# jw3il/graph-marl

Hardware: AMD Instinct MI355X
Metric: env-steps/sec (routing, --netmon, 20-node graphs) at 1/2/4/8 MI355X (higher is better)
Workload: dtype f32 (GEMMs: 3xf16-split MFMA, A low piece scaled 2^12, f32 accumulate); 1 GPU; routing rollout --netmon (NetMon K=1, H=128, enc 512,256, lstm, sum) + DQN 512,256 eps-greedy, random 20-node topologies, episode 50 steps; n_env_per_gpu=4096, n_nodes=20, n_data=20, gemm_form=x3, parallelism=dp1 (env shards, no rollout collective), stream_groups=2, graph_steps=10, resets_in_window=43

## Files before the change

### graph-marl_amd/_lib.py

```python
import ctypes as C
import os

import torch

HERE = os.path.dirname(os.path.abspath(__file__))
LIB_PATH = os.environ.get("GM_LIB") or os.path.join(HERE, "lib", "libgraphmarl_amd.so")

GM_OK = 0
GM_ERR_UNSUPPORTED = -5
GM_INFO_FIELDS = 9
INFO_KEYS = ["looped", "throughput", "dropped", "blocked", "n_delays", "sum_delays", "n_arrived",
             "sum_delays_arrived", "sum_spr"]
TOPO_FIXED, TOPO_RANDOM, TOPO_LIST, TOPO_SEQUENTIAL = 0, 1, 2, 3
GM_EVAL_FIELDS = 5
EVAL_KEYS = ["total_edge_load", "occupied_edges", "packets_on_edges", "total_packet_size", "sum_packet_distances"]

EXPORTS = [
    "gm_last_error", "gm_version", "gm_env_create", "gm_env_destroy", "gm_env_dims", "gm_env_reset",
    "gm_env_step", "gm_env_observe", "gm_env_topology", "gm_env_final_info", "gm_policy_egreedy", "gm_env_policy_step",
    "gm_env_get_state", "gm_env_set_state", "gm_build_seed_list", "gm_mp_aggregate", "gm_mp_aggregate_rows", "gm_mp_aggregate_bwd", "gm_leaky_bwd", "gm_netmon_readout",
    "gm_netmon_readout_bwd", "gm_netmon_readout_bwd_sym", "gm_lstm_pointwise", "gm_lstm_pointwise_bwd", "gm_linear_f32", "gm_gemm_f32",
    "gm_simple_create", "gm_simple_destroy", "gm_simple_reset", "gm_simple_step",
    "gm_simple_observe", "gm_simple_policy_egreedy", "gm_simple_get_state", "gm_env_set_topology",
    "gm_policy_shortest_path", "gm_env_first_hops", "gm_routing_node_encoder", "gm_gemm_x3", "gm_gemm_x3_head", "gm_absmax_scale", "gm_absmax_scale_rows", "gm_gemm_x3_wgrad", "gm_gemm_x3_wgrad2", "gm_absmax_finish",
    "gm_gemm_pack_x3", "gm_gemm_pack_x3_bytes", "gm_gemm_range_status",
    "gm_pcg64_seed", "gm_pcg64_choice", "gm_lnlstm_pointwise", "gm_agent_attention", "gm_agent_comm",
    "gm_gemm_x3_dgrad", "gm_lstm_cell_bwd", "gm_qhead_bwd", "gm_netmon_readout_ld", "gm_routing_node_encoder_bits", "gm_gather_records",
    "gm_lnlstm_fwd", "gm_lnlstm_bwd", "gm_gru_pointwise", "gm_gru_bwd", "gm_act_bwd", "gm_build_info",
    "gm_act_fwd", "gm_act_bwd_z", "gm_obs_from_gemm", "gm_encoder_x3", "gm_step_mse_blocks", "gm_step_mse",
    "gm_step_mse_bwd", "gm_gru_cell_fwd", "gm_gru_cell_bwd", "gm_lnlstm_cell_bwd", "gm_agent_comm_bwd",
    "gm_agent_attention_bwd", "gm_agent_attention_kl", "gm_netmon_global_rows", "gm_netmon_global_bwd",
]
TUNING_EXPORTS = ["gm_gemm_set_tile", "gm_gemm_set_wgrad", "gm_gemm_set_mfma", "gm_gemm_set_dgrad", "gm_gemm_form",
                  "gm_last_kernel", "gm_last_lnlstm_pw", "gm_gemm_kernel_name"]

GEMM_MODE = os.environ.get("GM_GEMM", "x3")
if GEMM_MODE not in ("x3", "f32"):
    raise ValueError(f"GM_GEMM must be 'x3' or 'f32', not {GEMM_MODE!r}")

class EnvConfig(C.Structure):
    _fields_ = [
        ("n_env", C.c_int32), ("n_nodes", C.c_int32), ("n_data", C.c_int32), ("env_var", C.c_int32),
        ("congestion", C.c_int32), ("action_mask", C.c_int32), ("ttl", C.c_int32), ("topo_mode", C.c_int32),
        ("topo_seed", C.c_int64), ("seed_list", C.POINTER(C.c_int64)), ("n_seed_list", C.c_int32),
        ("excluded", C.POINTER(C.c_int64)), ("n_excluded", C.c_int32), ("device", C.c_int32),
        ("k", C.c_int32),
    ]


class ObsBuffers(C.Structure):
    _fields_ = [("obs", C.c_void_p), ("obs_row_stride", C.c_int64), ("node_obs", C.c_void_p),
                ("agent_node", C.c_void_p), ("agent_adj", C.c_void_p), ("obs_gemm", C.c_void_p),
                ("obs_gemm_stride", C.c_int64)]


class StepDetail(C.Structure):
    _fields_ = [("done_steps", C.c_void_p), ("done_opt", C.c_void_p), ("success", C.c_void_p), ("eval", C.c_void_p)]


class EnvState(C.Structure):
    _fields_ = [(k, C.c_void_p) for k in [
        "now", "target", "edge", "time", "ttl", "start", "spw", "agent_steps", "size", "visited", "amask",
        "loads", "topo_seed", "topo_reps", "edge_a", "edge_b", "edge_len", "nbr_edge", "apsp", "rng_key",
        "rng_pos", "seq_index"]]


class PCG64(C.Structure):
# ... 61 lines not shown
def lib():
    global _lib
    if _lib is not None:
        return _lib
    if not os.path.exists(LIB_PATH):
        raise GMError(f"{LIB_PATH} not built: run `make -C graph-marl_amd/csrc` (or __graft_entry__.build())")
    L = C.CDLL(LIB_PATH)
    vp, i32, i64 = C.c_void_p, C.c_int32, C.c_int64
    L.gm_last_error.restype = C.c_char_p
    L.gm_env_create.argtypes = [C.POINTER(EnvConfig), vp, C.POINTER(vp)]
    L.gm_env_destroy.argtypes = [vp]
    L.gm_env_dims.argtypes = [vp] + [C.POINTER(i32)] * 5
    L.gm_env_reset.argtypes = [vp, vp, C.POINTER(ObsBuffers), vp]
    L.gm_env_step.argtypes = [vp, vp, vp, vp, vp, C.POINTER(StepDetail), C.POINTER(ObsBuffers), vp]
    L.gm_env_observe.argtypes = [vp, C.POINTER(ObsBuffers), vp]
    L.gm_env_topology.argtypes = [vp, vp, vp, vp, vp, vp]
    L.gm_env_final_info.argtypes = [vp, vp, vp]
    L.gm_policy_egreedy.argtypes = [vp, vp, C.c_double, vp, vp]
    L.gm_env_policy_step.argtypes = [vp, vp, C.c_double, vp, vp, vp, vp, C.POINTER(StepDetail), C.POINTER(ObsBuffers),
                                     vp]
    L.gm_env_get_state.argtypes = [vp, C.POINTER(EnvState)]
    L.gm_env_set_state.argtypes = [vp, C.POINTER(EnvState)]
    L.gm_build_seed_list.argtypes = [i32, i64, i32, vp, i32, i32, vp]
    L.gm_mp_aggregate.argtypes = [vp, vp, i32, i32, i32, i32, i32, vp, vp]
    L.gm_mp_aggregate_rows.argtypes = [vp, C.c_int64, vp, i32, i32, i32, i32, i32, vp, C.c_int64, vp]
    L.gm_leaky_bwd.argtypes = [vp, vp, C.c_int64, i32, C.c_float, vp, vp, i32, vp, vp]
    L.gm_mp_aggregate_bwd.argtypes = [vp, vp, i32, i32, i32, i32, i32, vp, vp]
    L.gm_netmon_readout.argtypes = [vp, vp, vp, vp, i32, i32, i32, i32, i32, vp, i64, vp]
    L.gm_netmon_readout_bwd.argtypes = [vp, i64, vp, vp, i32, i32, i32, i32, i32, vp, vp, vp]
    L.gm_lstm_pointwise.argtypes = [vp, vp, i32, i32, vp, vp, vp, vp]
    L.gm_lstm_pointwise_bwd.argtypes = [vp, vp, vp, vp, vp, i32, i32, vp, vp, vp, vp]
    L.gm_linear_f32.argtypes = [vp, i64, vp, i64, vp, i32, i32, i32, i32, vp, i64, vp]
    L.gm_gemm_set_tile.argtypes = [i32]
    L.gm_gemm_set_wgrad.argtypes = [i32]
    L.gm_gemm_set_mfma.argtypes = [i32]
    L.gm_gemm_set_dgrad.argtypes = [i32]
    L.gm_lstm_cell_bwd.argtypes = [C.POINTER(LSTMBwdArgs), vp]
    L.gm_qhead_bwd.argtypes = [vp, i64, i32, vp, i64, vp, i64, i64, i32, i32, vp, i64, vp, vp, vp, i32, vp, vp]
    L.gm_netmon_readout_ld.argtypes = [vp, i64, vp, i64, vp, vp, i32, i32, i32, i32, i32, vp, i64, vp]
    L.gm_routing_node_encoder_bits.argtypes = [vp, i64, vp, i32, i32, vp, vp, i32, i32, vp, i64, vp, i64, vp]
    L.gm_env_set_topology.argtypes = [vp, i32, i64, vp, i32, i32]
    L.gm_policy_shortest_path.argtypes = [vp, vp, vp]
    L.gm_env_first_hops.argtypes = [vp, vp, vp]
    L.gm_agent_attention.argtypes = [vp, vp, vp, i64, vp, i32, i32, i32, i32, i32, vp, i64, vp, vp]
    L.gm_agent_comm.argtypes = [vp, i64, vp, i32, i32, i32, vp, i64, vp]
    L.gm_gemm_pack_x3_bytes.argtypes = [i32, i32]
    L.gm_gemm_pack_x3_bytes.restype = i64
    L.gm_gemm_pack_x3.argtypes = [vp, i64, i32, i32, vp, vp, vp]
    L.gm_routing_node_encoder.argtypes = [vp, i64, vp, i32, i32, vp, vp, i32, i32, vp, i64, vp]
    L.gm_gemm_range_status.argtypes = [C.POINTER(i32), i32]
    L.gm_pcg64_seed.argtypes = [C.c_uint64, C.POINTER(PCG64)]
    L.gm_pcg64_choice.argtypes = [vp, i64, i64, vp, vp]
    L.gm_gather_records.argtypes = [vp, i64, i64, vp, vp, i32, i64, i64, vp, vp]
    L.gm_lnlstm_pointwise.argtypes = [vp, i64, vp, i64] + [vp] * 7 + [i32, i32, C.c_float, vp, i64, vp, i64, vp]
    newer = {
        "gm_lnlstm_fwd": [vp, i64, vp, i64, vp, i64] + [vp] * 7 + [i32, i32, C.c_float, vp, i64, vp, i64, vp, vp],
        "gm_lnlstm_bwd": [vp, i64, vp, i64, vp, i64] + [vp] * 8 + [vp, i64, vp, i64, i32, i32, i32, vp, i64, vp, i64, vp,
                                                                   i64, vp, vp],
        "gm_gru_pointwise": [vp, i64, vp, i64, vp, i64, i32, i32, vp, i64, vp],
        "gm_gru_bwd": [vp, i64, vp, i64, vp, i64, vp, i64, i32, i32, vp, i64, vp, i64, vp, i64, vp],
        "gm_act_bwd": [vp, vp, C.c_int64, i32, i32, vp, vp, i32, vp, vp],
        "gm_act_fwd": [vp, C.c_int64, i32, i32, vp, vp],
        "gm_act_bwd_z": [vp, vp, C.c_int64, i32, i32, vp, vp, i32, vp, vp],
        "gm_obs_from_gemm": [vp, i64, i64, i32, vp, i64, vp],
        "gm_step_mse_blocks": [i64],
        "gm_step_mse": [vp, vp, i64, i32, vp, vp],
# ... 167 lines not shown
```

### graph-marl_amd/csrc/gm_device.hpp

```cpp
#pragma once
#include <hip/hip_runtime.h>
#include <stdint.h>

void gm_set_last_kernel(const char* name);

namespace gm {

constexpr int WAVE = 64;
constexpr int MT_N = 624;
constexpr int MT_M = 397;
constexpr int MAX_NODES = 128;
constexpr int MAX_AGENTS = 64;
constexpr int MAX_KNBR = 8;
constexpr int MAX_EDGES = MAX_NODES * 3 / 2;
constexpr int RNG_BUF = 256;

__device__ __forceinline__ int lane_id() { return threadIdx.x; }

__device__ __forceinline__ int readlane(int v, int l) { return __builtin_amdgcn_readlane(v, l); }
__device__ __forceinline__ uint32_t readlane_u(uint32_t v, int l) {
    return (uint32_t)__builtin_amdgcn_readlane((int)v, l);
}
__device__ __forceinline__ double readlane_f64(double v, int l) {
    uint64_t b = __double_as_longlong(v);
    uint32_t lo = readlane_u((uint32_t)b, l), hi = readlane_u((uint32_t)(b >> 32), l);
    return __longlong_as_double((long long)(((uint64_t)hi << 32) | lo));
}
__device__ __forceinline__ uint64_t readlane_u64(uint64_t v, int l) {
    uint32_t lo = readlane_u((uint32_t)v, l), hi = readlane_u((uint32_t)(v >> 32), l);
    return ((uint64_t)hi << 32) | lo;
}
__device__ __forceinline__ uint64_t ballot(bool p) { return __ballot(p); }

__device__ __forceinline__ bool bit128(const uint64_t* m, int v) { return (m[v >> 6] >> (v & 63)) & 1ull; }
__device__ __forceinline__ void set128(uint64_t* m, int v) { m[v >> 6] |= 1ull << (v & 63); }

__device__ __forceinline__ uint64_t wave_or_u64(uint64_t v) {
    uint32_t lo = (uint32_t)v, hi = (uint32_t)(v >> 32);
#pragma unroll
    for (int m = 1; m < WAVE; m <<= 1) {
        lo |= (uint32_t)__shfl_xor((int)lo, m);
        hi |= (uint32_t)__shfl_xor((int)hi, m);
    }
    return ((uint64_t)hi << 32) | lo;
}
__device__ __forceinline__ int wave_sum_i32(int v) {
#pragma unroll
    for (int m = 1; m < WAVE; m <<= 1) v += __shfl_xor(v, m);
    return v;
}

__device__ __forceinline__ uint32_t mt_temper(uint32_t y) {
    y ^= (y >> 11);
    y ^= (y << 7) & 0x9d2c5680u;
    y ^= (y << 15) & 0xefc60000u;
    y ^= (y >> 18);
    return y;
}

__device__ __forceinline__ uint32_t mt_mix(uint32_t a, uint32_t b, uint32_t m) {
    uint32_t y = (a & 0x80000000u) | (b & 0x7fffffffu);
    return m ^ (y >> 1) ^ ((0u - (y & 1u)) & 0x9908b0dfu);
}

__device__ __forceinline__ void mt_twist_lds(uint32_t* k) {
    const int l = lane_id();
    for (int s = 0; s < MT_N; s += WAVE) {
        int i = s + l;
        uint32_t a = 0, b = 0, m = 0;
        if (i < MT_N) {
            a = k[i];
            b = k[i == MT_N - 1 ? 0 : i + 1];
            m = k[i < MT_N - MT_M ? i + MT_M : i - (MT_N - MT_M)];
        }
        __syncthreads();
        if (i < MT_N) k[i] = mt_mix(a, b, m);
        __syncthreads();
    }
}

__device__ __forceinline__ void mt_seed_lds(uint32_t* k, uint32_t seed, int n = MT_N) {
    if (lane_id() == 0) {
        uint32_t v = seed;
        k[0] = v;
        for (int i = 1; i < n; i++) {
            v = 1812433253u * (v ^ (v >> 30)) + (uint32_t)i;
            k[i] = v;
        }
    }
    __syncthreads();
}

__device__ __forceinline__ uint32_t mask_for(uint32_t rng) {
    uint32_t m = rng;
    m |= m >> 1; m |= m >> 2; m |= m >> 4; m |= m >> 8; m |= m >> 16;
    return m;
}

struct MainRng {
    uint32_t* g;
    uint32_t* buf;
    uint32_t* tmp;
    int cur, pos, has_next;
    int n, k;

    __device__ void twist_next() {
        const int l = lane_id();
        const uint32_t* src = g + cur * MT_N;
        for (int i = l; i < MT_N; i += WAVE) tmp[i] = src[i];
        __syncthreads();
        mt_twist_lds(tmp);
        uint32_t* dst = g + (1 - cur) * MT_N;
        for (int i = l; i < MT_N; i += WAVE) dst[i] = tmp[i];
        __syncthreads();
        has_next = 1;
    }
    __device__ void commit() {
        pos += k;
        n = 0;
        k = 0;
        if (pos >= MT_N && has_next) {
            pos -= MT_N;
            cur = 1 - cur;
            has_next = 0;
        }
    }
    __device__ void prefetch(int want) {
        commit();
        if (want > RNG_BUF) want = RNG_BUF;
        if (pos + want > MT_N && !has_next) twist_next();
        int avail = (MT_N - pos) + (has_next ? MT_N : 0);
        if (want > avail) want = avail;
        const int l = lane_id();
        for (int i = l; i < want; i += WAVE) {
            int o = pos + i;
            uint32_t w = o < MT_N ? g[cur * MT_N + o] : g[(1 - cur) * MT_N + (o - MT_N)];
            buf[i] = mt_temper(w);
        }
        __syncthreads();
        n = want;
    }
    __device__ __forceinline__ uint32_t next32() {
        if (k >= n) prefetch(RNG_BUF);
        return buf[k++];
    }
    __device__ __forceinline__ int64_t randint(int64_t high) {
        uint32_t rng = (uint32_t)(high - 1);
        if (rng == 0) return 0;
        uint32_t m = mask_for(rng), v;
        for (int guard = 0; (v = (next32() & m)) > rng; guard++)
            if (guard > 4096) return 0;
        return (int64_t)v;
    }
    __device__ __forceinline__ double random() {
        int32_t a = (int32_t)(next32() >> 5), b = (int32_t)(next32() >> 6);
        return (a * 67108864.0 + b) / 9007199254740992.0;
    }
};

struct LocalRng {
    uint32_t* key;
    int pos;
    int lim = MT_N;
    uint32_t sd = 0;
    __device__ void seed(uint32_t s) {
        mt_seed_lds(key, s);
        pos = MT_N;
        lim = MT_N;
        sd = s;
    }
    __device__ void seed_partial(uint32_t s, int w) {
        mt_seed_lds(key, s, MT_M + w);
        const int l = lane_id();
        for (int c = 0; c < w; c += WAVE) {
            const int i = c + l;
            uint32_t a = 0, b = 0, m = 0;
            if (i < w) {
                a = key[i];
                b = key[i + 1];
                m = key[i + MT_M];
            }
            __syncthreads();
            if (i < w) key[i] = mt_mix(a, b, m);
            __syncthreads();
        }
        pos = 0;
        lim = w;
        sd = s;
    }
    __device__ __forceinline__ uint32_t next32() {
        if (pos == MT_N) {
            mt_twist_lds(key);
            pos = 0;
        }
        if (pos >= lim) {
            mt_seed_lds(key, sd);
            mt_twist_lds(key);
            lim = MT_N;
        }
        return mt_temper(key[pos++]);
    }
    __device__ __forceinline__ int64_t randint(int64_t high) {
        uint32_t rng = (uint32_t)(high - 1);
        if (rng == 0) return 0;
        uint32_t m = mask_for(rng), v;
        for (int guard = 0; (v = (next32() & m)) > rng; guard++)
            if (guard > 4096) return 0;
        return (int64_t)v;
    }
};

}
```

### graph-marl_amd/csrc/gm_env.hip

```cpp
#include <hip/hip_runtime.h>

#include <algorithm>
#include <cstdio>
#include <cstring>
#include <string>
#include <vector>

#include "../../include/graph_marl_amd.h"
#include "gm_device.hpp"

using namespace gm;

namespace {
thread_local std::string g_err;
}

extern "C" const char* gm_last_error(void) { return g_err.c_str(); }
extern "C" int gm_version(void) { return 1; }

int gm_fail(int code, const std::string& msg) {
    g_err = msg;
    return code;
}

// ... 20 lines not shown
    uint64_t* visited;
    uint8_t* amask;
    double* load;
    uint32_t* mt;
    int32_t *mt_cur, *mt_pos, *mt_has_next;
    int32_t* err;
};

struct gm_env {
    gm_env_config cfg;
    std::vector<int64_t> list, excl;
    EnvDev d;
    std::vector<void*> allocs;
    int device;
};

namespace {

template <int NC>
struct EnvLds {
    int32_t now[MAX_AGENTS], target[MAX_AGENTS], edge[MAX_AGENTS], time[MAX_AGENTS];
    double size[MAX_AGENTS];
    double load[NC * 3 / 2];
    uint8_t nbr[NC * 3], nbr_edge[NC * 3];
    uint8_t ea[NC * 3 / 2], eb[NC * 3 / 2], elen[NC * 3 / 2];
    uint64_t nbrmask[NC][2];
    int8_t kn[MAX_AGENTS][MAX_KNBR];
    float node_cnt[NC], node_load[NC];
    alignas(16) uint32_t rbuf[RNG_BUF];
    uint32_t rtmp[MT_N];
};
constexpr int STG_FLOATS = RNG_BUF + MT_N;

template <class ES>
__device__ void load_topology_lds(const EnvDev& d, int env, ES& s) {
    const int l = lane_id();
    const int N = d.N, E = d.E;
    for (int i = l; i < N * 3; i += WAVE) {
        s.nbr[i] = (uint8_t)d.nbr[(size_t)env * N * 3 + i];
        s.nbr_edge[i] = (uint8_t)d.nbr_edge[(size_t)env * N * 3 + i];
    }
    for (int e = l; e < E; e += WAVE) {
        s.ea[e] = (uint8_t)d.edge_a[(size_t)env * E + e];
        s.eb[e] = (uint8_t)d.edge_b[(size_t)env * E + e];
        s.elen[e] = (uint8_t)d.edge_len[(size_t)env * E + e];
    }
    __syncthreads();
    for (int v = l; v < N; v += WAVE) {
        uint64_t m[2] = {0ull, 0ull};
        for (int k = 0; k < 3; k++) set128(m, s.nbr[v * 3 + k]);
        s.nbrmask[v][0] = m[0];
        s.nbrmask[v][1] = m[1];
    }
    __syncthreads();
}

template <class ES>
__device__ __forceinline__ MainRng open_rng(const EnvDev& d, int env, ES& s) {
    MainRng r;
    r.g = d.mt + (size_t)env * 2 * MT_N;
    r.buf = s.rbuf;
    r.tmp = s.rtmp;
    r.cur = d.mt_cur[env];
    r.pos = d.mt_pos[env];
    r.has_next = d.mt_has_next[env];
    r.n = 0;
    r.k = 0;
    return r;
}

__device__ __forceinline__ void close_rng(const EnvDev& d, int env, MainRng& r) {
    r.commit();
    if (lane_id() == 0) {
        d.mt_cur[env] = r.cur;
        d.mt_pos[env] = r.pos;
        d.mt_has_next[env] = r.has_next;
    }
}

__host__ __device__ __forceinline__ int obs_dim_of(int N, int env_var, int k) {
    return 6 * N + 10 + (env_var == 2 ? 5 * k : 0) + (env_var == 3 ? N * N + N * (4 * N + 8) : 0);
}

__device__ __forceinline__ void nbr_block(int r, int N, int& k, int& q) {
    k = (r >= N + 2) + (r >= 2 * (N + 2));
    q = r - k * (N + 2);
}
// ... 3 lines not shown
    const int nb = s.nbr[v * 3 + k], ne = s.nbr_edge[v * 3 + k];
    return q < N ? (float)(nb == q) : (q == N ? (float)s.elen[ne] : (float)s.load[ne]);
}

template <class ES>
__device__ __forceinline__ float node_obs_value(const ES& s, int N, int j, int c) {
    if (c < N) return (float)(c == j);
    if (c == N) return s.node_cnt[j];
    if (c == N + 1) return s.node_load[j];
    int k, q;
    nbr_block(c - (N + 2), N, k, q);
    return nbr_block_value(s, N, j, k, q);
}



template <class ES>
__device__ void emit_obs(const EnvDev& d, int env, ES& s, const gm_obs_buffers& o) {
    const int l = lane_id();
    const int N = d.N, A = d.A;
    if (o.node_obs || (o.obs && d.env_var == 3)) {
        for (int v = l; v < N; v += WAVE) {
            int cnt = 0;
            double tl = 0.0;
            for (int i = 0; i < A; i++) {
                if (s.now[i] == v && s.edge[i] == -1) {
                    cnt++;
                    tl += s.size[i];
                }
            }
            s.node_cnt[v] = (float)cnt;
            s.node_load[v] = (float)tl;
        }
        __syncthreads();
        if (o.node_obs) {
            const int ND = 4 * N + 8;
            float* base = o.node_obs + (size_t)env * N * ND;
            float* stg = reinterpret_cast<float*>(s.rbuf);
            const int per = STG_FLOATS / ND;
            const bool vec = (reinterpret_cast<uintptr_t>(base) & 15) == 0;
            for (int v0 = 0; v0 < N; v0 += per) {
                const int nr = min(per, N - v0), nf = nr * ND;
                for (int i = l; i < nf / 4; i += WAVE) reinterpret_cast<float4*>(stg)[i] = make_float4(0.f, 0.f, 0.f, 0.f);
                __syncthreads();
                if (l < nr) {
                    const int v = v0 + l;
                    float* row = stg + l * ND;
                    row[v] = 1.f;
                    row[N] = s.node_cnt[v];
                    row[N + 1] = s.node_load[v];
#pragma unroll
                    for (int k = 0; k < 3; k++) {
                        float* blk = row + N + 2 + k * (N + 2);
                        const int ne = s.nbr_edge[v * 3 + k];
                        blk[s.nbr[v * 3 + k]] = 1.f;
                        blk[N] = (float)s.elen[ne];
                        blk[N + 1] = (float)s.load[ne];
                    }
                }
                __syncthreads();
                float* dst = base + (size_t)v0 * ND;
                if (vec) {
                    for (int i = l; i < nf / 4; i += WAVE)
                        reinterpret_cast<float4*>(dst)[i] = reinterpret_cast<const float4*>(stg)[i];
                } else {
                    for (int i = l; i < nf; i += WAVE) dst[i] = stg[i];
                }
                __syncthreads();
            }
        }
    }
    if (o.obs && d.env_var == 2) {
        if (l < A) {
            const int now = s.now[l];
            int cnt = 0;
            for (int j = 0; j < A && cnt < d.k; j++) {
                if (j == l) continue;
                const int nj = s.now[j];
                if (nj == now || bit128(s.nbrmask[now], nj)) s.kn[l][cnt++] = (int8_t)j;
            }
            for (int q = cnt; q < d.k; q++) s.kn[l][q] = -1;
        }
        __syncthreads();
    }
    if (o.obs || o.obs_gemm) {
        const int D1 = 6 * N + 10, D = obs_dim_of(N, d.env_var, d.k);
        const size_t ld = o.obs_row_stride;
        float* base = o.obs ? o.obs + (size_t)env * A * ld : nullptr;
        float* stg = reinterpret_cast<float*>(s.rbuf);
        const int SR = (D1 + 3) & ~3, Q = D1 / 4, T = D1 - 4 * Q, per = STG_FLOATS / SR;
        const bool vec = (ld & 3) == 0 && (reinterpret_cast<uintptr_t>(base) & 15) == 0;
        for (int a0 = 0; a0 < A; a0 += per) {
            const int nr = min(per, A - a0);
            for (int i = l; i < nr * SR / 4; i += WAVE) reinterpret_cast<float4*>(stg)[i] = make_float4(0.f, 0.f, 0.f, 0.f);
            __syncthreads();
            if (l < nr) {
                const int a = a0 + l;
                float* row = stg + l * SR;
                const int now = s.now[a], e = s.edge[a];
                row[now] = 1.f;
                row[N + s.target[a]] = 1.f;
                row[2 * N] = (float)(e != -1);
                if (e >= 0) row[2 * N + 1 + (s.ea[e] ^ s.eb[e] ^ now)] = 1.f;
                row[3 * N + 1] = (float)s.time[a];
                row[3 * N + 2] = (float)s.size[a];
                row[3 * N + 3] = (float)a;
#pragma unroll
                for (int k = 0; k < 3; k++) {
                    float* blk = row + 3 * N + 4 + k * (N + 2);
                    const int ne = s.nbr_edge[now * 3 + k];
                    blk[s.nbr[now * 3 + k]] = 1.f;
                    blk[N] = (float)s.elen[ne];
                    blk[N + 1] = (float)s.load[ne];
                }
            }
            __syncthreads();
            if (!base) {
            } else if (vec) {
                const int Qr = Q + (T ? 1 : 0);
                for (int i = l; i < nr * Qr; i += WAVE) {
                    const int r = i / Qr, q = i - r * Qr;
                    const float4 v = *reinterpret_cast<const float4*>(stg + r * SR + 4 * q);
                    float* dst = base + (size_t)(a0 + r) * ld + 4 * q;
                    if (q < Q) {
                        *reinterpret_cast<float4*>(dst) = v;
                    } else if (T == 2) {
                        *reinterpret_cast<float2*>(dst) = make_float2(v.x, v.y);
                    } else {
                        for (int c = 0; c < T; c++) dst[c] = stg[r * SR + 4 * q + c];
                    }
                }
            } else {
                for (int i = l; i < nr * D1; i += WAVE) {
                    const int r = i / D1, c = i - r * D1;
                    base[(size_t)(a0 + r) * ld + c] = stg[r * SR + c];
                }
            }
            if (o.obs_gemm) {
                const int Qg = (D1 - 2) / 4;
                float* gb = o.obs_gemm + ((size_t)env * A + a0) * o.obs_gemm_stride;
                for (int i = l; i < nr * Qg; i += WAVE) {
                    const int r = i / Qg, q = i - r * Qg;
                    float v[4];
#pragma unroll
                    for (int j = 0; j < 4; j++) {
                        const int c = 4 * q + j;
                        v[j] = stg[r * SR + (c < N - 1 ? c : (c < 2 * N - 1 ? c + 1 : c + 2))];
                    }
                    *reinterpret_cast<float4*>(gb + (size_t)r * o.obs_gemm_stride + 4 * q) =
                        make_float4(v[0], v[1], v[2], v[3]);
                }
            }
            __syncthreads();
        }
        if (base && D > D1) {
            for (int a = 0; a < A; a++) {
                float* row = base + (size_t)a * ld;
                for (int c = D1 + l; c < D; c += WAVE) {
                    const int g = c - D1;
                    float v;
                    if (d.env_var == 2) {
                        const int slot = g / 5, f = g - slot * 5, j = s.kn[a][slot];
                        v = j < 0 ? -1.0f
                                  : f == 0 ? (float)s.now[j]
                                  : f == 1 ? (float)s.target[j]
                                  : f == 2 ? (float)s.edge[j]
                                  : f == 3 ? (float)s.size[j] : (float)a;
                    } else if (g < N * N) {
                        const int r = g / N, q = g - r * N;
                        v = (float)(r == q || bit128(s.nbrmask[r], q));
                    } else {
                        const int ND = 4 * N + 8, h = g - N * N, j = h / ND;
                        v = node_obs_value(s, N, j, h - j * ND);
                    }
                    row[c] = v;
                }
            }
        }
    }
    if (o.agent_node && l < A) o.agent_node[(size_t)env * A + l] = s.now[l];
    if (o.agent_adj) {
        int8_t* base = o.agent_adj + (size_t)env * A * A;
        for (int idx = l; idx < A * A; idx += WAVE) {
            int i = idx / A, j = idx - i * A;
            int ni = s.now[i], nj = s.now[j];
            base[idx] = (int8_t)(i == j || ni == nj || bit128(s.nbrmask[ni], nj));
        }
    }
}

template <class ES>
__device__ void load_packets_lds(const EnvDev& d, int env, ES& s) {
    const int l = lane_id();
    if (l < d.A) {
        size_t p = (size_t)env * d.A + l;
        s.now[l] = d.now[p];
        s.target[l] = d.target[p];
        s.edge[l] = d.edge[p];
        s.time[l] = d.time[p];
        s.size[l] = d.size[p];
    }
    for (int e = l; e < d.E; e += WAVE) s.load[e] = d.load[(size_t)env * d.E + e];
    __syncthreads();
}

template <int NC>
struct TopoLds {
    static constexpr int NCAP = NC;
    double x[NC], y[NC], d2[NC];
    uint32_t tkey[MT_N];
    int32_t deg[NC];
    uint64_t adj[NC][2];
    int32_t node_edges[NC * 3];
    int32_t ea[NC * 3 / 2], eb[NC * 3 / 2], elen[NC * 3 / 2];
    int32_t n_edges;
    int32_t cand_at_rank[NC];
    uint8_t ok_at_rank[NC];
};

__device__ __forceinline__ bool is_excluded(const EnvDev& d, int64_t sd) {
    int lo = 0, hi = d.n_excl - 1;
    while (lo <= hi) {
        int m = (lo + hi) >> 1;
        int64_t v = d.excl[m];
        if (v == sd) return true;
        if (v < sd) lo = m + 1;
        else hi = m - 1;
    }
    return false;
}

template <class R>
__device__ int64_t draw_topology_seed(const EnvDev& d, R& r) {
    int64_t sd = r.randint(2147483647LL);
    for (int guard = 0; d.n_excl > 0 && is_excluded(d, sd) && guard < 4096; guard++) sd = r.randint(2147483647LL);
    return sd;
// ... 389 lines not shown
    close_rng(d, env, r);
    if (l < A) {
        size_t p = (size_t)env * A + l;
        d.now[p] = p_now;
        d.target[p] = p_target;
        d.start[p] = p_now;
        d.size[p] = p_size;
        d.edge[p] = -1;
        d.time[p] = 0;
        d.ttl_[p] = d.ttl;
        d.steps[p] = 0;
        d.spw[p] = d.apsp[((size_t)env * N + p_now) * N + p_target];
        d.visited[p * 2 + 0] = p_now < 64 ? (1ull << p_now) : 0ull;
        d.visited[p * 2 + 1] = p_now >= 64 ? (1ull << (p_now - 64)) : 0ull;
        uint32_t m = d.amask_on ? (uint32_t)(p_now != p_target) : 0u;
        reinterpret_cast<uint32_t*>(d.amask)[p] = m;
        s.now[l] = p_now;
        s.target[l] = p_target;
        s.edge[l] = -1;
        s.time[l] = 0;
        s.size[l] = p_size;
    }
    for (int e = l; e < d.E; e += WAVE) {
        d.load[(size_t)env * d.E + e] = 0.0;
        s.load[e] = 0.0;
    }
    __syncthreads();
    if (o.obs || o.obs_gemm || o.node_obs || o.agent_node || o.agent_adj) {
        load_topology_lds(d, env, s);
        emit_obs(d, env, s, o);
    }
}

__device__ __forceinline__ int egreedy_lane(const EnvDev& d, const float* q, double eps, size_t p,
                                            const uint32_t* rbuf, int l, int A) {
    const float4 qv = reinterpret_cast<const float4*>(q)[p];
    float v[4] = {qv.x, qv.y, qv.z, qv.w};
    if (d.amask_on) {
        const uint32_t m = reinterpret_cast<const uint32_t*>(d.amask)[p];
        for (int k = 0; k < 4; k++)
            if ((m >> (8 * k)) & 0xffu) v[k] = -__builtin_inff();
    }
    int best = 0;
    for (int k = 1; k < 4; k++)
        if (v[k] > v[best]) best = k;
    const int ra = (int)(rbuf[l] & 3u);
    const uint32_t w0 = rbuf[A + 2 * l], w1 = rbuf[A + 2 * l + 1];
    const double u = ((int32_t)(w0 >> 5) * 67108864.0 + (int32_t)(w1 >> 6)) / 9007199254740992.0;
    return u < eps ? ra : best;
}

struct StepOut {
    float* reward;
    uint8_t* done;
    double* info;
    gm_step_detail det;
    const float* q;
    double eps;
    int32_t* act_out;
};

template <int NC>
__global__ __launch_bounds__(64) void k_env_step(EnvDev d, const int32_t* act, StepOut out, gm_obs_buffers o) {
    const int env = blockIdx.x;
    const int l = lane_id();
    const int N = d.N, A = d.A, E = d.E;
    __shared__ EnvLds<NC> s;
    load_topology_lds(d, env, s);

    const bool own = l < A;
    const size_t p = (size_t)env * A + l;
    int now = 0, target = 0, edge = -1, time = 0, ttl = 0, steps = 0, spw = 0, start = 0, a_t = 0;
    double size = 0.0;
    uint64_t vis[2] = {0ull, 0ull};
    int rng_cur = 0, rng_pos = 0, rng_next = 0;
    const bool pol = out.q != nullptr;
    if (pol) {
        MainRng r = open_rng(d, env, s);
        r.prefetch(3 * A);
        if (own) a_t = egreedy_lane(d, out.q, out.eps, p, s.rbuf, l, A);
        r.k = 3 * A;
        close_rng(d, env, r);
        rng_cur = r.cur;
        rng_pos = r.pos;
        rng_next = r.has_next;
        if (own) out.act_out[p] = a_t;
    }
    if (own) {
        now = d.now[p]; target = d.target[p]; edge = d.edge[p]; time = d.time[p];
        ttl = d.ttl_[p]; steps = d.steps[p]; spw = d.spw[p]; start = d.start[p];
        size = d.size[p]; vis[0] = d.visited[p * 2]; vis[1] = d.visited[p * 2 + 1];
        if (!pol) a_t = act[p];
        if (a_t < 0 || a_t > 3) {
            atomicExch(d.err, GM_ERR_INVALID_ARG);
            a_t = 0;
        }
    }
    double ld0 = l < E ? d.load[(size_t)env * E + l] : 0.0;
    double ld1 = l + WAVE < E ? d.load[(size_t)env * E + l + WAVE] : 0.0;
    double ld2 = l + 2 * WAVE < E ? d.load[(size_t)env * E + l + 2 * WAVE] : 0.0;

    steps += 1;
    float reward = 0.0f;

    int chosen = -1;
    if (own && edge == -1 && a_t != 0) chosen = s.nbr_edge[now * 3 + (a_t - 1)];
    uint64_t admit = 0, block = 0;
    for (int i = 0; i < A; i++) {
        int c = readlane(chosen, i);
        if (c < 0) continue;
        double si = readlane_f64(size, i);
        if ((c & (WAVE - 1)) == l) {
            const int slot = c >> 6;
            double ld = slot == 0 ? ld0 : (slot == 1 ? ld1 : ld2);
            if (d.cong && ld + si > 1.0) {
                block |= 1ull << i;
            } else {
                ld = ld + si;
                admit |= 1ull << i;
                if (slot == 0) ld0 = ld;
                else if (slot == 1) ld1 = ld;
                else ld2 = ld;
            }
        }
    }
    admit = wave_or_u64(admit);
    block = wave_or_u64(block);
    bool looped = false;
    if (own) {
        if ((block >> l) & 1ull) reward = reward - 0.2f;
        if ((admit >> l) & 1ull) {
            edge = chosen;
            time = s.elen[chosen];
            now = s.ea[chosen] ^ s.eb[chosen] ^ now;
            if (bit128(vis, now)) looped = true;
            else set128(vis, now);
        }
    }

    if (out.det.eval) {
        double tel = 0.0, tps = 0.0;
        int occ = 0;
        for (int e = 0; e < E; e++) {
            double le = e < WAVE ? readlane_f64(ld0, e)
                                 : (e < 2 * WAVE ? readlane_f64(ld1, e - WAVE) : readlane_f64(ld2, e - 2 * WAVE));
            tel = tel + le;
            occ += le > 0.0;
        }
        for (int i = 0; i < A; i++) tps = tps + readlane_f64(size, i);
        const int on_edges = __popcll(ballot(own && edge != -1));
        const int dist = wave_sum_i32(own ? (int)d.apsp[((size_t)env * N + now) * N + target] : 0);
        if (l == 0) {
            double* ev = out.det.eval + (size_t)env * GM_EVAL_FIELDS;
            ev[GM_EVAL_TOTAL_EDGE_LOAD] = tel;
            ev[GM_EVAL_OCCUPIED_EDGES] = (double)occ;
            ev[GM_EVAL_PACKETS_ON_EDGES] = (double)on_edges;
            ev[GM_EVAL_TOTAL_PACKET_SIZE] = tps;
            ev[GM_EVAL_SUM_PACKET_DISTANCES] = (double)dist;
        }
    }

    int sub_edge = -1;
    bool drop = false, fin = false, reached = false;
    uint32_t am = 0;
    if (own) {
        am = reinterpret_cast<const uint32_t*>(d.amask)[p];
        ttl -= 1;
        if (edge != -1) {
            time -= 1;
            if (time <= 0) {
                sub_edge = edge;
                edge = -1;
            }
        }
        drop = d.ttl > 0 && ttl <= 0;
        if (d.amask_on) {
            if (edge != -1) {
                am = 0;
            } else {
                am = 1u;
                int cnt = 1;
                for (int k = 0; k < 3; k++) {
                    uint32_t b = (uint32_t)bit128(vis, s.nbr[now * 3 + k]);
                    am |= b << (8 * (k + 1));
                    cnt += (int)b;
                }
                if (cnt == 4) drop = true;
            }
        }
        reached = edge == -1 && now == target;
        fin = reached || drop;
        if (fin) {
            reward = reward + (reached ? 10.0f : -10.0f);
            if (edge != -1) sub_edge = edge;
        }
    }
    for (int i = 0; i < A; i++) {
        int c = readlane(sub_edge, i);
        if (c < 0) continue;
// ... 7 lines not shown
    uint64_t finm = ballot(own && fin);
    uint64_t succm = ballot(own && fin && reached);
    uint64_t loopm = ballot(own && looped);
    if (out.det.done_steps && own) out.det.done_steps[p] = done_steps;
    if (out.det.done_opt && own) out.det.done_opt[p] = fin ? opt : 0;
    if (out.det.success && own) out.det.success[p] = (uint8_t)(fin && reached);
    if (out.info) {
        int sd = wave_sum_i32(fin ? steps : 0);
        int sda = wave_sum_i32(fin && reached ? steps : 0);
        double spr_sum = 0.0;
        for (int i = 0; i < A; i++) {
            if (!((succm >> i) & 1ull)) continue;
            int st = readlane(steps, i), op = readlane(opt, i);
            spr_sum += (double)st / (double)op;
        }
        if (l == 0) {
            double* inf = out.info + (size_t)env * GM_INFO_FIELDS;
            inf[GM_INFO_LOOPED] = (double)__popcll(loopm);
            inf[GM_INFO_THROUGHPUT] = (double)__popcll(succm);
            inf[GM_INFO_DROPPED] = (double)__popcll(finm & ~succm);
            inf[GM_INFO_BLOCKED] = (double)__popcll(block);
            inf[GM_INFO_N_DELAYS] = (double)__popcll(finm);
            inf[GM_INFO_SUM_DELAYS] = (double)sd;
            inf[GM_INFO_N_ARRIVED] = (double)__popcll(succm);
            inf[GM_INFO_SUM_DELAYS_ARRIVED] = (double)sda;
            inf[GM_INFO_SUM_SPR] = spr_sum;
        }
    }
    if (own) {
        out.reward[p] = reward;
        out.done[p] = (uint8_t)fin;
    }
    if (finm) {
        MainRng r = open_rng(d, env, s);
        if (pol) {
            r.cur = rng_cur;
            r.pos = rng_pos;
            r.has_next = rng_next;
        }
        r.prefetch(6 * __popcll(finm) + 8);
        uint64_t m = finm;
        while (m) {
            int i = __builtin_ctzll(m);
            m &= m - 1;
            int st = (int)r.randint(N);
            int tg = (int)r.randint(N);
            double sz = r.random();
            if (l == i) {
                now = st;
                target = tg;
                size = sz;
                start = st;
            }
        }
        close_rng(d, env, r);
        if (own && fin) {
            time = 0;
            edge = -1;
            ttl = d.ttl;
            steps = 0;
            spw = d.apsp[((size_t)env * N + now) * N + target];
            vis[0] = 0ull;
            vis[1] = 0ull;
            set128(vis, now);
            am = d.amask_on ? (uint32_t)(now != target) : 0u;
        }
    }
    if (own) {
        d.now[p] = now; d.target[p] = target; d.edge[p] = edge; d.time[p] = time;
        d.ttl_[p] = ttl; d.steps[p] = steps; d.spw[p] = spw; d.start[p] = start;
        d.size[p] = size; d.visited[p * 2] = vis[0]; d.visited[p * 2 + 1] = vis[1];
        reinterpret_cast<uint32_t*>(d.amask)[p] = am;
        s.now[l] = now; s.target[l] = target; s.edge[l] = edge; s.time[l] = time; s.size[l] = size;
    }
    if (l < E) { d.load[(size_t)env * E + l] = ld0; s.load[l] = ld0; }
    if (l + WAVE < E) { d.load[(size_t)env * E + l + WAVE] = ld1; s.load[l + WAVE] = ld1; }
    if (l + 2 * WAVE < E) { d.load[(size_t)env * E + l + 2 * WAVE] = ld2; s.load[l + 2 * WAVE] = ld2; }
    __syncthreads();
    if (o.obs || o.obs_gemm || o.node_obs || o.agent_node || o.agent_adj) emit_obs(d, env, s, o);
}

template <int NC>
__global__ __launch_bounds__(64) void k_env_observe(EnvDev d, gm_obs_buffers o) {
    const int env = blockIdx.x;
    __shared__ EnvLds<NC> s;
    load_topology_lds(d, env, s);
    load_packets_lds(d, env, s);
    emit_obs(d, env, s, o);
}

__global__ __launch_bounds__(256) void k_obs_from_gemm(const float* __restrict__ g, long long ldg, long long rows, int N,
                                                       float* __restrict__ obs, long long ldo) {
    const long long r = (long long)blockIdx.x * 4 + (threadIdx.x >> 6);
    if (r >= rows) return;
    const int l = threadIdx.x & 63;
    const float* gr = g + r * ldg;
    float* orow = obs + r * ldo;
    const int D1 = 6 * N + 10, Q = (D1 + 3) / 4;
    float pos = 0.f, tgt = 0.f, hop = 0.f;
    for (int c = l; c < N - 1; c += 64) pos += gr[c];
    for (int c = N - 1 + l; c < 2 * N - 1; c += 64) tgt += gr[c];
    for (int c = 2 * N - 1 + l; c < 3 * N - 1; c += 64) hop += gr[c];
#pragma unroll
    for (int o = 32; o > 0; o >>= 1) {
        pos += __shfl_xor(pos, o);
        tgt += __shfl_xor(tgt, o);
        hop += __shfl_xor(hop, o);
    }
    for (int q = l; q < Q; q += 64) {
        float v[4];
#pragma unroll
// ... 366 lines not shown

extern "C" int gm_env_dims(const gm_env* env, int32_t* n_env, int32_t* n_nodes, int32_t* n_data, int32_t* obs_dim,
                           int32_t* node_obs_dim) {
    if (!env) return gm_fail(GM_ERR_INVALID_ARG, "null env");
    if (n_env) *n_env = env->d.n_env;
    if (n_nodes) *n_nodes = env->d.N;
    if (n_data) *n_data = env->d.A;
    if (obs_dim) *obs_dim = obs_dim_of(env->d.N, env->d.env_var, env->d.k);
    if (node_obs_dim) *node_obs_dim = 4 * env->d.N + 8;
    return GM_OK;
}

static int check_obs(const gm_env* env, const gm_obs_buffers* o) {
    if (o && o->obs && o->obs_row_stride < obs_dim_of(env->d.N, env->d.env_var, env->d.k))
        return gm_fail(GM_ERR_INVALID_ARG, "obs_row_stride smaller than the observation size");
    if (o && o->obs_gemm &&
        (env->d.env_var != 1 || (env->d.N & 1) || o->obs_gemm_stride < 6 * env->d.N + 8 ||
         (o->obs_gemm_stride % 4) || (reinterpret_cast<uintptr_t>(o->obs_gemm) & 15)))
        return gm_fail(GM_ERR_INVALID_ARG, "obs_gemm: env_var 1, even N, stride >= 6N+8 and 16-byte rows");
    return GM_OK;
}

extern "C" int gm_env_reset(gm_env* env, const uint8_t* reset_mask, const gm_obs_buffers* obs, void* stream) {
    if (!env) return gm_fail(GM_ERR_INVALID_ARG, "null env");
    int rc = check_obs(env, obs);
    if (rc) return rc;
    gm_obs_buffers o = obs ? *obs : gm_obs_buffers{};
    if (env->d.N <= 32) hipLaunchKernelGGL(k_env_reset<32>, dim3(env->d.n_env), dim3(64), 0, (hipStream_t)stream, env->d, reset_mask, o);
    else if (ncap(env->d.N) == 64) hipLaunchKernelGGL(k_env_reset<64>, dim3(env->d.n_env), dim3(64), 0, (hipStream_t)stream, env->d, reset_mask, o);
    else hipLaunchKernelGGL(k_env_reset<128>, dim3(env->d.n_env), dim3(64), 0, (hipStream_t)stream, env->d, reset_mask, o);
    return check_launch();
}

static int launch_step(gm_env* env, const int32_t* actions, const float* q, double epsilon, int32_t* act_out,
                       float* reward, uint8_t* done, double* info, const gm_step_detail* detail,
                       const gm_obs_buffers* obs, void* stream) {
    int rc = check_obs(env, obs);
    if (rc) return rc;
    StepOut so;
    so.reward = reward;
    so.done = done;
    so.info = info;
    so.det = detail ? *detail : gm_step_detail{};
    so.q = q;
    so.eps = epsilon;
    so.act_out = act_out;
    gm_obs_buffers o = obs ? *obs : gm_obs_buffers{};
    if (ncap(env->d.N) == 64) hipLaunchKernelGGL(k_env_step<64>, dim3(env->d.n_env), dim3(64), 0, (hipStream_t)stream, env->d, actions, so, o);
    else hipLaunchKernelGGL(k_env_step<128>, dim3(env->d.n_env), dim3(64), 0, (hipStream_t)stream, env->d, actions, so, o);
    return check_launch();
}

extern "C" int gm_env_step(gm_env* env, const int32_t* actions, float* reward, uint8_t* done, double* info,
                           const gm_step_detail* detail, const gm_obs_buffers* obs, void* stream) {
    if (!env || !actions || !reward || !done) return gm_fail(GM_ERR_INVALID_ARG, "null argument");
    return launch_step(env, actions, nullptr, 0.0, nullptr, reward, done, info, detail, obs, stream);
}

extern "C" int gm_env_policy_step(gm_env* env, const float* q, double epsilon, int32_t* actions, float* reward,
                                  uint8_t* done, double* info, const gm_step_detail* detail, const gm_obs_buffers* obs,
                                  void* stream) {
    if (!env || !q || !actions || !reward || !done) return gm_fail(GM_ERR_INVALID_ARG, "null argument");
    if ((reinterpret_cast<uintptr_t>(q) & 15) != 0) return gm_fail(GM_ERR_INVALID_ARG, "q must be 16-byte aligned");
    return launch_step(env, nullptr, q, epsilon, actions, reward, done, info, detail, obs, stream);
}

__global__ void k_topology_rewind(EnvDev d, int interleave) {
    const int env = blockIdx.x * blockDim.x + threadIdx.x;
    if (env >= d.n_env) return;
    d.seq_index[env] = interleave ? env % d.n_list : 0;
    d.topo_ready[env] = 0;
}

extern "C" int gm_policy_shortest_path(gm_env* env, int32_t* actions, void* stream) {
    if (!env || !actions) return gm_fail(GM_ERR_INVALID_ARG, "gm_policy_shortest_path: null argument");
    if (ncap(env->d.N) == 64) hipLaunchKernelGGL(k_policy_shortest_path<64>, dim3(env->d.n_env), dim3(64), 0, (hipStream_t)stream, env->d, actions);
    else hipLaunchKernelGGL(k_policy_shortest_path<128>, dim3(env->d.n_env), dim3(64), 0, (hipStream_t)stream, env->d, actions);
    return check_launch();
}

extern "C" int gm_env_first_hops(gm_env* env, int32_t* out, void* stream) {
    if (!env || !out) return gm_fail(GM_ERR_INVALID_ARG, "gm_env_first_hops: null argument");
    if (ncap(env->d.N) == 64) hipLaunchKernelGGL(k_env_first_hops<64>, dim3(env->d.n_env), dim3(64), 0, (hipStream_t)stream, env->d, out);
// ... 230 lines not shown
```

### include/graph_marl_amd_tuning.h

```cpp
#pragma once
#include <stdint.h>
#ifdef __cplusplus
extern "C" {
#endif

int gm_gemm_set_wgrad(int32_t form);
int gm_gemm_set_tile(int32_t tile);
int gm_gemm_set_mfma(int32_t shape);
int gm_gemm_set_dgrad(int32_t form);
const char* gm_gemm_form(void);
const char* gm_last_kernel(void);
const char* gm_last_lnlstm_pw(void);
const char* gm_gemm_kernel_name(int32_t i);

#ifdef __cplusplus
}
#endif
```

Before: 6.973 million env-steps/s.

## Pack multiple envs per block in env step kernel with wave-level sync

The env step kernel now runs several environments per workgroup, one wavefront each with its own LDS slot, instead of one 64-thread block per env. Block-wide __syncthreads calls in the RNG and observation helpers become wavefront-scoped fences and barriers. The topology load is split into a register fetch issued early and an LDS commit later, so its latency overlaps with state and q loads. The RNG is opened once and reused across the policy and reset phases. The aim is to cut launch and scheduling overhead and expose more memory-level parallelism. The cost is higher LDS use per block, and correctness now depends on each env being touched only by its own wavefront.

```diff
diff --git a/graph-marl_amd/_lib.py b/graph-marl_amd/_lib.py
--- a/graph-marl_amd/_lib.py
+++ b/graph-marl_amd/_lib.py
@@ -32,7 +32,7 @@
     "gm_agent_attention_bwd", "gm_agent_attention_kl", "gm_netmon_global_rows", "gm_netmon_global_bwd",
 ]
 TUNING_EXPORTS = ["gm_gemm_set_tile", "gm_gemm_set_wgrad", "gm_gemm_set_mfma", "gm_gemm_set_dgrad", "gm_gemm_form",
-                  "gm_last_kernel", "gm_last_lnlstm_pw", "gm_gemm_kernel_name"]
+                  "gm_last_kernel", "gm_last_lnlstm_pw", "gm_gemm_kernel_name", "gm_env_set_step_epb"]
 
 GEMM_MODE = os.environ.get("GM_GEMM", "x3")
 if GEMM_MODE not in ("x3", "f32"):
@@ -160,6 +160,8 @@
     L.gm_lstm_pointwise_bwd.argtypes = [vp, vp, vp, vp, vp, i32, i32, vp, vp, vp, vp]
     L.gm_linear_f32.argtypes = [vp, i64, vp, i64, vp, i32, i32, i32, i32, vp, i64, vp]
     L.gm_gemm_set_tile.argtypes = [i32]
+    if hasattr(L, "gm_env_set_step_epb"):
+        L.gm_env_set_step_epb.argtypes = [i32]
     L.gm_gemm_set_wgrad.argtypes = [i32]
     L.gm_gemm_set_mfma.argtypes = [i32]
     L.gm_gemm_set_dgrad.argtypes = [i32]
diff --git a/graph-marl_amd/csrc/gm_device.hpp b/graph-marl_amd/csrc/gm_device.hpp
--- a/graph-marl_amd/csrc/gm_device.hpp
+++ b/graph-marl_amd/csrc/gm_device.hpp
@@ -15,7 +15,17 @@
 constexpr int MAX_EDGES = MAX_NODES * 3 / 2;
 constexpr int RNG_BUF = 256;
 
-__device__ __forceinline__ int lane_id() { return threadIdx.x; }
+__device__ __forceinline__ int lane_id() { return threadIdx.x & (WAVE - 1); }
+
+__device__ __forceinline__ void wave_sync() {
+    __builtin_amdgcn_fence(__ATOMIC_RELEASE, "workgroup");
+    __builtin_amdgcn_wave_barrier();
+    __builtin_amdgcn_fence(__ATOMIC_ACQUIRE, "workgroup");
+}
+__device__ __forceinline__ void lds_sync() {
+    __builtin_amdgcn_fence(__ATOMIC_ACQ_REL, "wavefront");
+    __builtin_amdgcn_wave_barrier();
+}
 
 __device__ __forceinline__ int readlane(int v, int l) { return __builtin_amdgcn_readlane(v, l); }
 __device__ __forceinline__ uint32_t readlane_u(uint32_t v, int l) {
@@ -73,9 +83,9 @@
             b = k[i == MT_N - 1 ? 0 : i + 1];
             m = k[i < MT_N - MT_M ? i + MT_M : i - (MT_N - MT_M)];
         }
-        __syncthreads();
+        wave_sync();
         if (i < MT_N) k[i] = mt_mix(a, b, m);
-        __syncthreads();
+        wave_sync();
     }
 }
 
@@ -88,7 +98,7 @@
             k[i] = v;
         }
     }
-    __syncthreads();
+    wave_sync();
 }
 
 __device__ __forceinline__ uint32_t mask_for(uint32_t rng) {
@@ -108,11 +118,11 @@
         const int l = lane_id();
         const uint32_t* src = g + cur * MT_N;
         for (int i = l; i < MT_N; i += WAVE) tmp[i] = src[i];
-        __syncthreads();
+        wave_sync();
         mt_twist_lds(tmp);
         uint32_t* dst = g + (1 - cur) * MT_N;
         for (int i = l; i < MT_N; i += WAVE) dst[i] = tmp[i];
-        __syncthreads();
+        wave_sync();
         has_next = 1;
     }
     __device__ void commit() {
@@ -137,7 +147,7 @@
             uint32_t w = o < MT_N ? g[cur * MT_N + o] : g[(1 - cur) * MT_N + (o - MT_N)];
             buf[i] = mt_temper(w);
         }
-        __syncthreads();
+        wave_sync();
         n = want;
     }
     __device__ __forceinline__ uint32_t next32() {
@@ -180,9 +190,9 @@
                 b = key[i + 1];
                 m = key[i + MT_M];
             }
-            __syncthreads();
+            wave_sync();
             if (i < w) key[i] = mt_mix(a, b, m);
-            __syncthreads();
+            wave_sync();
         }
         pos = 0;
         lim = w;
diff --git a/graph-marl_amd/csrc/gm_env.hip b/graph-marl_amd/csrc/gm_env.hip
--- a/graph-marl_amd/csrc/gm_env.hip
+++ b/graph-marl_amd/csrc/gm_env.hip
@@ -76,27 +76,68 @@
 };
 constexpr int STG_FLOATS = RNG_BUF + MT_N;
 
-template <class ES>
-__device__ void load_topology_lds(const EnvDev& d, int env, ES& s) {
+template <int NC>
+struct TopoRegs {
+    static constexpr int TN = (NC * 3 + WAVE - 1) / WAVE, TE = (NC * 3 / 2 + WAVE - 1) / WAVE;
+    int32_t nbr[TN], nbr_edge[TN], ea[TE], eb[TE], elen[TE];
+};
+
+template <int NC>
+__device__ __forceinline__ void topology_fetch(const EnvDev& d, int env, TopoRegs<NC>& t) {
     const int l = lane_id();
     const int N = d.N, E = d.E;
-    for (int i = l; i < N * 3; i += WAVE) {
-        s.nbr[i] = (uint8_t)d.nbr[(size_t)env * N * 3 + i];
-        s.nbr_edge[i] = (uint8_t)d.nbr_edge[(size_t)env * N * 3 + i];
-    }
-    for (int e = l; e < E; e += WAVE) {
-        s.ea[e] = (uint8_t)d.edge_a[(size_t)env * E + e];
-        s.eb[e] = (uint8_t)d.edge_b[(size_t)env * E + e];
-        s.elen[e] = (uint8_t)d.edge_len[(size_t)env * E + e];
-    }
-    __syncthreads();
+    const size_t bn = (size_t)env * N * 3, be = (size_t)env * E;
+#pragma unroll
+    for (int j = 0; j < TopoRegs<NC>::TN; j++) {
+        const int i = l + j * WAVE;
+        t.nbr[j] = i < N * 3 ? d.nbr[bn + i] : 0;
+        t.nbr_edge[j] = i < N * 3 ? d.nbr_edge[bn + i] : 0;
+    }
+#pragma unroll
+    for (int j = 0; j < TopoRegs<NC>::TE; j++) {
+        const int e = l + j * WAVE;
+        t.ea[j] = e < E ? d.edge_a[be + e] : 0;
+        t.eb[j] = e < E ? d.edge_b[be + e] : 0;
+        t.elen[j] = e < E ? d.edge_len[be + e] : 0;
+    }
+}
+
+template <int NC, class ES>
+__device__ __forceinline__ void topology_commit(const EnvDev& d, const TopoRegs<NC>& t, ES& s) {
+    const int l = lane_id();
+    const int N = d.N, E = d.E;
+#pragma unroll
+    for (int j = 0; j < TopoRegs<NC>::TN; j++) {
+        const int i = l + j * WAVE;
+        if (i < N * 3) {
+            s.nbr[i] = (uint8_t)t.nbr[j];
+            s.nbr_edge[i] = (uint8_t)t.nbr_edge[j];
+        }
+    }
+#pragma unroll
+    for (int j = 0; j < TopoRegs<NC>::TE; j++) {
+        const int e = l + j * WAVE;
+        if (e < E) {
+            s.ea[e] = (uint8_t)t.ea[j];
+            s.eb[e] = (uint8_t)t.eb[j];
+            s.elen[e] = (uint8_t)t.elen[j];
+        }
+    }
+    lds_sync();
     for (int v = l; v < N; v += WAVE) {
         uint64_t m[2] = {0ull, 0ull};
         for (int k = 0; k < 3; k++) set128(m, s.nbr[v * 3 + k]);
         s.nbrmask[v][0] = m[0];
         s.nbrmask[v][1] = m[1];
     }
-    __syncthreads();
+    lds_sync();
+}
+
+template <int NC>
+__device__ void load_topology_lds(const EnvDev& d, int env, EnvLds<NC>& s) {
+    TopoRegs<NC> t;
+    topology_fetch(d, env, t);
+    topology_commit(d, t, s);
 }
 
 template <class ES>
@@ -166,7 +207,7 @@
             s.node_cnt[v] = (float)cnt;
             s.node_load[v] = (float)tl;
         }
-        __syncthreads();
+        lds_sync();
         if (o.node_obs) {
             const int ND = 4 * N + 8;
             float* base = o.node_obs + (size_t)env * N * ND;
@@ -176,7 +217,7 @@
             for (int v0 = 0; v0 < N; v0 += per) {
                 const int nr = min(per, N - v0), nf = nr * ND;
                 for (int i = l; i < nf / 4; i += WAVE) reinterpret_cast<float4*>(stg)[i] = make_float4(0.f, 0.f, 0.f, 0.f);
-                __syncthreads();
+                lds_sync();
                 if (l < nr) {
                     const int v = v0 + l;
                     float* row = stg + l * ND;
@@ -192,7 +233,7 @@
                         blk[N + 1] = (float)s.load[ne];
                     }
                 }
-                __syncthreads();
+                lds_sync();
                 float* dst = base + (size_t)v0 * ND;
                 if (vec) {
                     for (int i = l; i < nf / 4; i += WAVE)
@@ -200,7 +241,7 @@
                 } else {
                     for (int i = l; i < nf; i += WAVE) dst[i] = stg[i];
                 }
-                __syncthreads();
+                lds_sync();
             }
         }
     }
@@ -215,7 +256,7 @@
             }
             for (int q = cnt; q < d.k; q++) s.kn[l][q] = -1;
         }
-        __syncthreads();
+        lds_sync();
     }
     if (o.obs || o.obs_gemm) {
         const int D1 = 6 * N + 10, D = obs_dim_of(N, d.env_var, d.k);
@@ -227,7 +268,7 @@
         for (int a0 = 0; a0 < A; a0 += per) {
             const int nr = min(per, A - a0);
             for (int i = l; i < nr * SR / 4; i += WAVE) reinterpret_cast<float4*>(stg)[i] = make_float4(0.f, 0.f, 0.f, 0.f);
-            __syncthreads();
+            lds_sync();
             if (l < nr) {
                 const int a = a0 + l;
                 float* row = stg + l * SR;
@@ -248,7 +289,7 @@
                     blk[N + 1] = (float)s.load[ne];
                 }
             }
-            __syncthreads();
+            lds_sync();
             if (!base) {
             } else if (vec) {
                 const int Qr = Q + (T ? 1 : 0);
@@ -285,7 +326,7 @@
                         make_float4(v[0], v[1], v[2], v[3]);
                 }
             }
-            __syncthreads();
+            lds_sync();
         }
         if (base && D > D1) {
             for (int a = 0; a < A; a++) {
@@ -335,7 +376,7 @@
         s.size[l] = d.size[p];
     }
     for (int e = l; e < d.E; e += WAVE) s.load[e] = d.load[(size_t)env * d.E + e];
-    __syncthreads();
+    lds_sync();
 }
 
 template <int NC>
@@ -791,12 +832,10 @@
     }
 }
 
-__device__ __forceinline__ int egreedy_lane(const EnvDev& d, const float* q, double eps, size_t p,
-                                            const uint32_t* rbuf, int l, int A) {
-    const float4 qv = reinterpret_cast<const float4*>(q)[p];
+__device__ __forceinline__ int egreedy_pick(const EnvDev& d, float4 qv, uint32_t m, double eps, const uint32_t* rbuf,
+                                            int l, int A) {
     float v[4] = {qv.x, qv.y, qv.z, qv.w};
     if (d.amask_on) {
-        const uint32_t m = reinterpret_cast<const uint32_t*>(d.amask)[p];
         for (int k = 0; k < 4; k++)
             if ((m >> (8 * k)) & 0xffu) v[k] = -__builtin_inff();
     }
@@ -807,6 +846,12 @@
     const uint32_t w0 = rbuf[A + 2 * l], w1 = rbuf[A + 2 * l + 1];
     const double u = ((int32_t)(w0 >> 5) * 67108864.0 + (int32_t)(w1 >> 6)) / 9007199254740992.0;
     return u < eps ? ra : best;
+}
+__device__ __forceinline__ int egreedy_lane(const EnvDev& d, const float* q, double eps, size_t p,
+                                            const uint32_t* rbuf, int l, int A) {
+    const float4 qv = reinterpret_cast<const float4*>(q)[p];
+    const uint32_t m = d.amask_on ? reinterpret_cast<const uint32_t*>(d.amask)[p] : 0u;
+    return egreedy_pick(d, qv, m, eps, rbuf, l, A);
 }
 
 struct StepOut {
@@ -819,45 +864,51 @@
     int32_t* act_out;
 };
 
-template <int NC>
-__global__ __launch_bounds__(64) void k_env_step(EnvDev d, const int32_t* act, StepOut out, gm_obs_buffers o) {
-    const int env = blockIdx.x;
+template <int NC, int EPB>
+__global__ __launch_bounds__(64 * EPB) void k_env_step(EnvDev d, const int32_t* act, StepOut out, gm_obs_buffers o) {
+    const int wv = __builtin_amdgcn_readfirstlane((int)(threadIdx.x >> 6));
+    const int env = blockIdx.x * EPB + wv;
+    if (env >= d.n_env) return;
     const int l = lane_id();
     const int N = d.N, A = d.A, E = d.E;
-    __shared__ EnvLds<NC> s;
-    load_topology_lds(d, env, s);
-
+    __shared__ EnvLds<NC> sh[EPB];
+    EnvLds<NC>& s = sh[wv];
+
+    const bool pol = out.q != nullptr;
     const bool own = l < A;
     const size_t p = (size_t)env * A + l;
+    MainRng r = open_rng(d, env, s);
+    TopoRegs<NC> topo;
+    topology_fetch(d, env, topo);
     int now = 0, target = 0, edge = -1, time = 0, ttl = 0, steps = 0, spw = 0, start = 0, a_t = 0;
     double size = 0.0;
     uint64_t vis[2] = {0ull, 0ull};
-    int rng_cur = 0, rng_pos = 0, rng_next = 0;
-    const bool pol = out.q != nullptr;
-    if (pol) {
-        MainRng r = open_rng(d, env, s);
-        r.prefetch(3 * A);
-        if (own) a_t = egreedy_lane(d, out.q, out.eps, p, s.rbuf, l, A);
-        r.k = 3 * A;
-        close_rng(d, env, r);
-        rng_cur = r.cur;
-        rng_pos = r.pos;
-        rng_next = r.has_next;
-        if (own) out.act_out[p] = a_t;
-    }
+    uint32_t am = 0;
+    float4 qv = make_float4(0.f, 0.f, 0.f, 0.f);
+    if (own && pol) qv = reinterpret_cast<const float4*>(out.q)[p];
+    if (own && !pol) a_t = act[p];
     if (own) {
         now = d.now[p]; target = d.target[p]; edge = d.edge[p]; time = d.time[p];
         ttl = d.ttl_[p]; steps = d.steps[p]; spw = d.spw[p]; start = d.start[p];
         size = d.size[p]; vis[0] = d.visited[p * 2]; vis[1] = d.visited[p * 2 + 1];
-        if (!pol) a_t = act[p];
-        if (a_t < 0 || a_t > 3) {
-            atomicExch(d.err, GM_ERR_INVALID_ARG);
-            a_t = 0;
-        }
+        am = reinterpret_cast<const uint32_t*>(d.amask)[p];
     }
     double ld0 = l < E ? d.load[(size_t)env * E + l] : 0.0;
     double ld1 = l + WAVE < E ? d.load[(size_t)env * E + l + WAVE] : 0.0;
     double ld2 = l + 2 * WAVE < E ? d.load[(size_t)env * E + l + 2 * WAVE] : 0.0;
+
+    if (pol) {
+        r.prefetch(3 * A);
+        if (own) a_t = egreedy_pick(d, qv, am, out.eps, s.rbuf, l, A);
+        r.k = 3 * A;
+        close_rng(d, env, r);
+        if (own) out.act_out[p] = a_t;
+    }
+    topology_commit(d, topo, s);
+    if (own && (a_t < 0 || a_t > 3)) {
+        atomicExch(d.err, GM_ERR_INVALID_ARG);
+        a_t = 0;
+    }
 
     steps += 1;
     float reward = 0.0f;
@@ -921,9 +972,7 @@
 
     int sub_edge = -1;
     bool drop = false, fin = false, reached = false;
-    uint32_t am = 0;
     if (own) {
-        am = reinterpret_cast<const uint32_t*>(d.amask)[p];
         ttl -= 1;
         if (edge != -1) {
             time -= 1;
@@ -997,12 +1046,6 @@
         out.done[p] = (uint8_t)fin;
     }
     if (finm) {
-        MainRng r = open_rng(d, env, s);
-        if (pol) {
-            r.cur = rng_cur;
-            r.pos = rng_pos;
-            r.has_next = rng_next;
-        }
         r.prefetch(6 * __popcll(finm) + 8);
         uint64_t m = finm;
         while (m) {
@@ -1041,7 +1084,7 @@
     if (l < E) { d.load[(size_t)env * E + l] = ld0; s.load[l] = ld0; }
     if (l + WAVE < E) { d.load[(size_t)env * E + l + WAVE] = ld1; s.load[l + WAVE] = ld1; }
     if (l + 2 * WAVE < E) { d.load[(size_t)env * E + l + 2 * WAVE] = ld2; s.load[l + 2 * WAVE] = ld2; }
-    __syncthreads();
+    lds_sync();
     if (o.obs || o.obs_gemm || o.node_obs || o.agent_node || o.agent_adj) emit_obs(d, env, s, o);
 }
 
@@ -1474,6 +1517,17 @@
     return check_launch();
 }
 
+constexpr int STEP_EPB_DEFAULT = 4;
+static int g_step_epb = -1;
+
+template <int EPB>
+static void launch_step_kernel(bool small, const EnvDev& d, const int32_t* actions, const StepOut& so,
+                               const gm_obs_buffers& o, hipStream_t stream) {
+    const dim3 grid((unsigned)((d.n_env + EPB - 1) / EPB)), block(64 * EPB);
+    if (small) hipLaunchKernelGGL((k_env_step<64, EPB>), grid, block, 0, stream, d, actions, so, o);
+    else hipLaunchKernelGGL((k_env_step<128, EPB>), grid, block, 0, stream, d, actions, so, o);
+}
+
 static int launch_step(gm_env* env, const int32_t* actions, const float* q, double epsilon, int32_t* act_out,
                        float* reward, uint8_t* done, double* info, const gm_step_detail* detail,
                        const gm_obs_buffers* obs, void* stream) {
@@ -1488,9 +1542,19 @@
     so.eps = epsilon;
     so.act_out = act_out;
     gm_obs_buffers o = obs ? *obs : gm_obs_buffers{};
-    if (ncap(env->d.N) == 64) hipLaunchKernelGGL(k_env_step<64>, dim3(env->d.n_env), dim3(64), 0, (hipStream_t)stream, env->d, actions, so, o);
-    else hipLaunchKernelGGL(k_env_step<128>, dim3(env->d.n_env), dim3(64), 0, (hipStream_t)stream, env->d, actions, so, o);
+    const int epb = g_step_epb > 0 ? g_step_epb : STEP_EPB_DEFAULT;
+    const bool small = ncap(env->d.N) == 64;
+    if (epb == 1) launch_step_kernel<1>(small, env->d, actions, so, o, (hipStream_t)stream);
+    else if (epb == 2) launch_step_kernel<2>(small, env->d, actions, so, o, (hipStream_t)stream);
+    else launch_step_kernel<4>(small, env->d, actions, so, o, (hipStream_t)stream);
     return check_launch();
+}
+
+extern "C" int gm_env_set_step_epb(int32_t epb) {
+    if (epb != -1 && epb != 1 && epb != 2 && epb != 4)
+        return gm_fail(GM_ERR_INVALID_ARG, "gm_env_set_step_epb: envs per block in {-1, 1, 2, 4}");
+    g_step_epb = epb;
+    return GM_OK;
 }
 
 extern "C" int gm_env_step(gm_env* env, const int32_t* actions, float* reward, uint8_t* done, double* info,
diff --git a/include/graph_marl_amd_tuning.h b/include/graph_marl_amd_tuning.h
--- a/include/graph_marl_amd_tuning.h
+++ b/include/graph_marl_amd_tuning.h
@@ -11,6 +11,7 @@
 const char* gm_gemm_form(void);
 const char* gm_last_kernel(void);
 const char* gm_last_lnlstm_pw(void);
+int gm_env_set_step_epb(int32_t epb);
 const char* gm_gemm_kernel_name(int32_t i);
 
 #ifdef __cplusplus
```

After: 6.989 million env-steps/s (median of 2 runs). Within noise of the previous version (+0.2%).
